# zju3dv/LoG

Hardware: NVIDIA H100
Metric: gaussians_per_s_fwd_bwd (higher is better)
Workload: dtype f32

## Files before the change

### log_b200/csrc/lgr_bin.cu

```cuda
#include "lgr_common.cuh"
#include "lgr_prof.cuh"

namespace lgr {

constexpr int SCAN_THREADS = 1024;
constexpr int SORT_CAP_SMALL_FWD = 4096;

__global__ void __launch_bounds__(SCAN_THREADS)
tile_scan_kernel(int ntiles, int32_t* __restrict__ tile_start ,
                 int32_t* __restrict__ cursor ,
                 int32_t* __restrict__ meta, int small_cap) {
  __shared__ int warp_sum[SCAN_THREADS / 32];
  __shared__ int carry_s, maxl_s, nbig_s;
  const int tid = threadIdx.x, lane = tid & 31, wid = tid >> 5;
  if (tid == 0) { carry_s = 0; maxl_s = 0; nbig_s = 0; }
  __syncthreads();
  int local_max = 0;
  for (int base = 0; base < ntiles; base += SCAN_THREADS) {
    const int i = base + tid;
    const int c = (i < ntiles) ? cursor[i * CSTRIDE] + cursor[i * CSTRIDE + 1] : 0;
    local_max = max(local_max, c);
    int x = c;
#pragma unroll
    for (int o = 1; o < 32; o <<= 1) { const int y = __shfl_up_sync(0xffffffffu, x, o); if (lane >= o) x += y; }
    if (lane == 31) warp_sum[wid] = x;
    __syncthreads();
    if (wid == 0) {
      int w = warp_sum[lane];
#pragma unroll
      for (int o = 1; o < 32; o <<= 1) { const int y = __shfl_up_sync(0xffffffffu, w, o); if (lane >= o) w += y; }
      warp_sum[lane] = w;
    }
    __syncthreads();
    const int carry = carry_s;
    const int excl = carry + (wid ? warp_sum[wid - 1] : 0) + x - c;
    if (i < ntiles) {
      tile_start[i] = excl; cursor[i * CSTRIDE] = 0;
      if (c > small_cap) cursor[CSTRIDE * ntiles + atomicAdd(&nbig_s, 1)] = i;
    }
    __syncthreads();
    if (tid == SCAN_THREADS - 1) carry_s = carry + warp_sum[31];
    __syncthreads();
  }
#pragma unroll
  for (int o = 16; o > 0; o >>= 1) local_max = max(local_max, __shfl_xor_sync(0xffffffffu, local_max, o));
  if (lane == 0) atomicMax(&maxl_s, local_max);
  __syncthreads();
  if (tid == 0) { tile_start[ntiles] = carry_s; meta[0] = carry_s; meta[1] = maxl_s; meta[5] = nbig_s; }
}

constexpr int BIN_THREADS = 256;
constexpr int PART_ROUNDS = 8;
constexpr int PLACE_GRID = 132 * 4;
constexpr int PART_CAP = 2048;
constexpr int PART_FLUSH_AT = PART_CAP - 4 * BIN_THREADS;
constexpr int PLACE_ITEMS = 8;
constexpr int PLACE_CHUNK = PLACE_ITEMS * BIN_THREADS;
#ifndef LGR_BIN_DIRECT_MAX
#define LGR_BIN_DIRECT_MAX (1 << 16)
#endif
constexpr int64_t BIN_DIRECT_MAX = LGR_BIN_DIRECT_MAX;
constexpr int PLACE_WINDOW = 2047;

__device__ __forceinline__ unsigned long long composite(uint32_t k, uint32_t v) { return ((unsigned long long)k << 32) | v; }

int part_smem_bytes(int rows) { return 3 * (int)sizeof(int32_t) * max(rows, 1); }

__device__ __forceinline__ void block_exclusive_scan(const int* in, int* out, int len, int* wsum) {
  const int tid = threadIdx.x, lane = tid & 31, wid = tid >> 5;
  int carry = 0;
  for (int base = 0; base < len; base += BIN_THREADS) {
    const int c = base + tid < len ? in[base + tid] : 0;
    int x = c;
#pragma unroll
    for (int o = 1; o < 32; o <<= 1) { const int y = __shfl_up_sync(0xffffffffu, x, o); if (lane >= o) x += y; }
    if (lane == 31) wsum[wid] = x;
    __syncthreads();
    int before = carry, all = carry;
#pragma unroll
    for (int w = 0; w < BIN_THREADS / 32; w++) { if (w < wid) before += wsum[w]; all += wsum[w]; }
    if (base + tid < len) out[base + tid] = before + x - c;
    carry = all;
    __syncthreads();
  }
}

__global__ void __launch_bounds__(BIN_THREADS, 6)
bin_partition_kernel(View v, int64_t n, const float* __restrict__ splat, const int32_t* __restrict__ radii,
                     const int32_t* __restrict__ tile_start, int32_t* __restrict__ cursor, unsigned long long* __restrict__ stage,
                     int32_t* __restrict__ stage_tile, int64_t capacity ,
                     int rounds ,
                     uint32_t* __restrict__ direct_key, uint32_t* __restrict__ direct_val ) {
  extern __shared__ int32_t row_tab[];
  __shared__ uint32_t s_key[PART_CAP], s_id[PART_CAP];
  __shared__ int32_t s_tile[PART_CAP];
  __shared__ uint16_t s_perm[PART_CAP];
  __shared__ int s_fill;
  __shared__ int s_wsum[BIN_THREADS / 32];
  __shared__ int64_t s_first[LGR_SHARD_MAX_RANKS + 1];
  const int rows = v.row1 - v.row0, lane = threadIdx.x & 31;
  int32_t* r_cnt = row_tab;
  int32_t* r_off = row_tab + rows;
  int32_t* r_base = row_tab + 2 * rows;
  for (int r = threadIdx.x; r < rows; r += BIN_THREADS) r_cnt[r] = 0;
  if (threadIdx.x == 0) s_fill = 0;
  const int64_t total = v.region_count ? region_setup(v, s_first) : n;
  __syncthreads();
  auto flush = [&]() {
    const int held = s_fill;
    if (direct_key) {
      for (int e = threadIdx.x; e < held; e += BIN_THREADS) {
        const int t = s_tile[e];
        const int64_t pos = (int64_t)tile_start[t] + atomicAdd(cursor + t * CSTRIDE, 1);
        if (pos < capacity) { direct_key[pos] = s_key[e]; direct_val[pos] = s_id[e]; }
      }
      __syncthreads();
      for (int r = threadIdx.x; r < rows; r += BIN_THREADS) r_cnt[r] = 0;
      if (threadIdx.x == 0) s_fill = 0;
      __syncthreads();
      return;
    }
    for (int r = threadIdx.x; r < rows; r += BIN_THREADS) {
      const int c = r_cnt[r];
      if (c > 0) r_base[r] = tile_start[r * v.gx] + atomicAdd(cursor + r * v.gx * CSTRIDE + 2, c);
    }
    block_exclusive_scan(r_cnt, r_off, rows, s_wsum);
    for (int r = threadIdx.x; r < rows; r += BIN_THREADS) r_base[r] -= r_off[r];
    __syncthreads();
    for (int e = threadIdx.x; e < held; e += BIN_THREADS) s_perm[atomicAdd(&r_off[s_tile[e] / v.gx], 1)] = (uint16_t)e;
    __syncthreads();
    for (int j = threadIdx.x; j < held; j += BIN_THREADS) {
      const int e = s_perm[j], t = s_tile[e];
      const int64_t pos = (int64_t)r_base[t / v.gx] + j;
      if (pos < capacity) { stage[pos] = composite(s_key[e], s_id[e]); stage_tile[pos] = t; }
    }
    __syncthreads();
    for (int r = threadIdx.x; r < rows; r += BIN_THREADS) r_cnt[r] = 0;
    if (threadIdx.x == 0) s_fill = 0;
    __syncthreads();
  };
  for (int64_t chunk = (int64_t)blockIdx.x * rounds * BIN_THREADS; chunk < total; chunk += (int64_t)gridDim.x * rounds * BIN_THREADS) {
    for (int round = 0; round < rounds; round++) {
      int64_t i = chunk + round * BIN_THREADS + threadIdx.x;
      bool live = i < total;
      if (live && v.region_count) i = region_row(v, s_first, i);
      if (live && v.num_owners > 0) {
        const int b = (int)(i / 256), sl = (int)(i % 256);
        if (sl >= v.band_blk[b]) live = false;
        else {
          const int id = v.band_ids[i];
          v.band_rows[v.band_blk[v.band_blocks + b] + sl] = id;
          if (v.band_dsplat) {
            float4* z = reinterpret_cast<float4*>(v.band_dsplat + (int64_t)id * LGR_GRAD_FLOATS);
            z[0] = z[1] = z[2] = make_float4(0.f, 0.f, 0.f, 0.f);
          }
          i = id;
        }
      }
      int rad = 0;
      float4 r0 = make_float4(0.f, 0.f, 0.f, 0.f), r1 = r0;
      float depth = 0.f;
      if (live) {
        rad = radii[i];
        r0 = ldg4(splat + i * LGR_SPLAT_FLOATS);
        r1 = ldg4(splat + i * LGR_SPLAT_FLOATS + 4);
        depth = __ldg(splat + i * LGR_SPLAT_FLOATS + 11);
        live = rad > 0;
      }
      if (live && v.num_owners == 0 && v.band_dsplat) {
        float4* z = reinterpret_cast<float4*>(v.band_dsplat + i * LGR_GRAD_FLOATS);
        z[0] = z[1] = z[2] = make_float4(0.f, 0.f, 0.f, 0.f);
      }
      int x0 = 0, y0 = 0, x1 = 0, y1 = 0;
      uint32_t key = 0;
      if (live) {
        live = r1.z > 0.f;
        if (live) {
          key = __float_as_uint(depth);
          tile_rect_tight(r0.x, r0.y, rad, r1.z, r1.w, v.gx, v.gy, v.row0, v.row1, x0, y0, x1, y1);
        }
      }
      const int w = x1 - x0, cnt = live ? w * (y1 - y0) : 0;
      const int mine = cnt <= 4 ? cnt : 0;
      int incl = mine;
#pragma unroll
      for (int o = 1; o < 32; o <<= 1) { const int y = __shfl_up_sync(0xffffffffu, incl, o); if (lane >= o) incl += y; }
      int wbase = 0;
      if (lane == 31 && incl > 0) wbase = atomicAdd(&s_fill, incl);
      wbase = __shfl_sync(0xffffffffu, wbase, 31);
      for (int k = 0, s = wbase + incl - mine; k < mine; k++, s++) {
        const int ty = y0 + k / w, tx = x0 + k % w;
        s_key[s] = key; s_id[s] = (uint32_t)i; s_tile[s] = (ty - v.row0) * v.gx + tx;
        atomicAdd(&r_cnt[ty - v.row0], 1);
      }
      unsigned todo = __ballot_sync(0xffffffffu, cnt > 4);
      while (todo) {
        const int src = __ffs(todo) - 1;
        todo &= todo - 1;
        const int bx0 = __shfl_sync(0xffffffffu, x0, src), by0 = __shfl_sync(0xffffffffu, y0, src);
        const int bw = __shfl_sync(0xffffffffu, w, src), bcnt = __shfl_sync(0xffffffffu, cnt, src);
        const uint32_t bkey = __shfl_sync(0xffffffffu, key, src);
        const uint32_t bid = (uint32_t)__shfl_sync(0xffffffffu, (int)i, src);
        const int bh = bcnt / bw;
        if (direct_key) {
          for (int k = lane; k < bcnt; k += 32) {
            const int t = (by0 + k / bw - v.row0) * v.gx + bx0 + k % bw;
            const int64_t pos = (int64_t)tile_start[t] + atomicAdd(cursor + t * CSTRIDE, 1);
            if (pos < capacity) { direct_key[pos] = bkey; direct_val[pos] = bid; }
          }
          continue;
        }
        for (int ry = 0; ry < bh; ry += 32) {
          const int nr = min(32, bh - ry), r_lane = by0 + ry + lane - v.row0;
          int rb = 0;
          if (lane < nr) rb = tile_start[r_lane * v.gx] + atomicAdd(cursor + r_lane * v.gx * CSTRIDE + 2, bw);
          for (int k0 = 0; k0 < nr * bw; k0 += 32) {
            const int k = k0 + lane;
            const int p = __shfl_sync(0xffffffffu, rb, k < nr * bw ? k / bw : 0);
            if (k < nr * bw) {
              const int64_t pos = (int64_t)p + k % bw;
              if (pos < capacity) {
                stage[pos] = composite(bkey, bid);
                stage_tile[pos] = (by0 + ry + k / bw - v.row0) * v.gx + bx0 + k % bw;
              }
            }
          }
        }
      }
      __syncthreads();
      if (__syncthreads_or(s_fill > (round == rounds - 1 ? 0 : PART_FLUSH_AT))) flush();
    }
  }
}

__global__ void __launch_bounds__(BIN_THREADS)
bin_place_kernel(int gx, int ntiles, const int32_t* __restrict__ tile_start, int32_t* __restrict__ cursor,
                 const unsigned long long* __restrict__ stage, const int32_t* __restrict__ stage_tile, uint32_t* __restrict__ inst_key,
                 uint32_t* __restrict__ inst_val) {
  constexpr int PER = (PLACE_WINDOW + 1) / BIN_THREADS;
  static_assert(PER * BIN_THREADS == PLACE_WINDOW + 1, "bucket count");
  __shared__ int s_cnt[PLACE_WINDOW + 1];
  __shared__ int s_base[PLACE_WINDOW];
  __shared__ unsigned long long s_e[PLACE_CHUNK];
  __shared__ uint16_t s_b[PLACE_CHUNK];
  __shared__ int s_wsum[BIN_THREADS / 32];
  __shared__ int s_t0;
  const int lane = threadIdx.x & 31, wid = threadIdx.x >> 5;
  const int total = tile_start[ntiles];
  for (int beg = blockIdx.x * PLACE_CHUNK; beg < total; beg += gridDim.x * PLACE_CHUNK) {
    for (int j = threadIdx.x; j <= PLACE_WINDOW; j += BIN_THREADS) s_cnt[j] = 0;
    if (threadIdx.x == 0) s_t0 = stage_tile[beg] - stage_tile[beg] % gx;
    __syncthreads();
    const int t0 = s_t0;
    int tk[PLACE_ITEMS], rank[PLACE_ITEMS];
#pragma unroll
    for (int k = 0; k < PLACE_ITEMS; k++) {
      const int idx = beg + k * BIN_THREADS + threadIdx.x;
      tk[k] = idx < total ? stage_tile[idx] : -1;
    }
#pragma unroll
    for (int k = 0; k < PLACE_ITEMS; k++) {
      rank[k] = 0;
      if (tk[k] >= 0) {
        const int b = min(tk[k] - t0, PLACE_WINDOW);
        rank[k] = b < PLACE_WINDOW ? atomicAdd(&s_cnt[b], 1) : tile_start[tk[k]] + atomicAdd(cursor + tk[k] * CSTRIDE, 1);
        tk[k] = b;
      }
    }
    __syncthreads();
    int c[PER], sum = 0;
    const int b0 = threadIdx.x * PER;
    int32_t* const cur = cursor + (int64_t)(t0 + b0) * CSTRIDE;
#pragma unroll
    for (int q = 0; q < PER; q++) {
      c[q] = s_cnt[b0 + q];
      sum += c[q];
    }
#pragma unroll
    for (int q = 0; q < PER; q++)
      if (c[q] > 0 && b0 + q < PLACE_WINDOW) s_base[b0 + q] = tile_start[t0 + b0 + q] + atomicAdd(cur + q * CSTRIDE, c[q]);
    int x = sum;
#pragma unroll
    for (int o = 1; o < 32; o <<= 1) { const int y = __shfl_up_sync(0xffffffffu, x, o); if (lane >= o) x += y; }
    if (lane == 31) s_wsum[wid] = x;
    __syncthreads();
    int off = x - sum;
#pragma unroll
    for (int w = 0; w < BIN_THREADS / 32; w++) if (w < wid) off += s_wsum[w];
#pragma unroll
    for (int q = 0; q < PER; q++) {
      const int b = threadIdx.x * PER + q;
      s_cnt[b] = off;
      if (b < PLACE_WINDOW && c[q] > 0) s_base[b] -= off;
      off += c[q];
    }
    __syncthreads();
#pragma unroll
    for (int k = 0; k < PLACE_ITEMS; k++) {
      if (tk[k] >= 0) {
        const unsigned long long e = stage[beg + k * BIN_THREADS + threadIdx.x];
        const int b = tk[k];
        if (b < PLACE_WINDOW) {
          const int j = s_cnt[b] + rank[k];
          s_e[j] = e; s_b[j] = (uint16_t)b;
        } else {
          inst_key[rank[k]] = (uint32_t)(e >> 32); inst_val[rank[k]] = (uint32_t)e;
        }
      }
    }
    __syncthreads();
    const int inside = s_cnt[PLACE_WINDOW];
    for (int j = threadIdx.x; j < inside; j += BIN_THREADS) {
      const int pos = s_base[s_b[j]] + j;
      const unsigned long long e = s_e[j];
      inst_key[pos] = (uint32_t)(e >> 32); inst_val[pos] = (uint32_t)e;
    }
    __syncthreads();
  }
}

constexpr int SORT_THREADS = 256;
constexpr int SORT_WARPS = SORT_THREADS / 32;
constexpr int RADIX_BITS = 8;
constexpr int RADIX = 1 << RADIX_BITS;
constexpr int SORT_CAP_SMALL = SORT_CAP_SMALL_FWD;
constexpr int SORT_CAP_LARGE = 13312;

__device__ __forceinline__ bool radix_pass(const uint32_t* __restrict__ kin, const uint32_t* __restrict__ vin,
                                           uint32_t* __restrict__ kout, uint32_t* __restrict__ vout, int len, int shift,
                                           bool on_val, int* __restrict__ whist) {
  const int tid = threadIdx.x, lane = tid & 31, wid = tid >> 5;
  const int seg = ((len + SORT_WARPS * 32 - 1) / (SORT_WARPS * 32)) * 32;
  const int beg = min(len, wid * seg), end = min(len, beg + seg);
  for (int j = tid; j < SORT_WARPS * RADIX; j += SORT_THREADS) whist[j] = 0;
  __syncthreads();
  int* myh = whist + wid * RADIX;
  for (int i = beg + lane; i < end; i += 32) {
    const uint32_t d = ((on_val ? vin[i] : kin[i]) >> shift) & (RADIX - 1);
    atomicAdd(myh + d, 1);
  }
  __syncthreads();
  {
    const int d = tid;
    int tot = 0;
#pragma unroll
    for (int w = 0; w < SORT_WARPS; w++) tot += whist[w * RADIX + d];
    int x = tot;
#pragma unroll
    for (int o = 1; o < 32; o <<= 1) { const int y = __shfl_up_sync(0xffffffffu, x, o); if (lane >= o) x += y; }
    __shared__ int wsum[SORT_WARPS];
    if (lane == 31) wsum[wid] = x;
    __syncthreads();
    int base = x - tot;
#pragma unroll
    for (int w = 0; w < SORT_WARPS; w++) if (w < wid) base += wsum[w];
#pragma unroll
    for (int w = 0; w < SORT_WARPS; w++) { const int c = whist[w * RADIX + d]; whist[w * RADIX + d] = base; base += c; }
    if (__syncthreads_or(tot == len)) return true;
  }
  for (int i0 = beg; i0 < end; i0 += 32) {
    const int i = i0 + lane;
    const bool ok = i < end;
    uint32_t k = 0, val = 0;
    if (ok) { k = kin[i]; val = vin[i]; }
    const uint32_t d = ok ? (((on_val ? val : k) >> shift) & (RADIX - 1)) : (RADIX + lane);
    const uint32_t peers = __match_any_sync(0xffffffffu, d);
    const int rank = __popc(peers & ((1u << lane) - 1u));
    int base = 0;
    if (ok) base = myh[d];
    __syncwarp();
    if (ok && rank == 0) myh[d] = base + __popc(peers);
    __syncwarp();
    if (ok) { kout[base + rank] = k; vout[base + rank] = val; }
  }
  __syncthreads();
  return false;
}

__device__ __forceinline__ void sort_tile(uint32_t* kA, uint32_t* vA, uint32_t* kB, uint32_t* vB, int len, int id_bits,
                                          int* whist) {
  uint32_t *ki = kA, *vi = vA, *ko = kB, *vo = vB;
  auto run = [&](int shift, bool on_val) {
    const bool ident = radix_pass(ki, vi, ko, vo, len, shift, on_val, whist);
    if (!ident) { uint32_t* t = ki; ki = ko; ko = t; t = vi; vi = vo; vo = t; }
  };
  for (int s = 0; s < 32; s += RADIX_BITS) run(s, false);
  int my_tie = 0;
  for (int i = threadIdx.x + 1; i < len; i += SORT_THREADS) if (ki[i] == ki[i - 1]) my_tie = 1;
  if (__syncthreads_or(my_tie)) {
    for (int s = 0; s < id_bits; s += RADIX_BITS) run(s, true);
    for (int s = 0; s < 32; s += RADIX_BITS) run(s, false);
  }
  if (ki != kA) {
    for (int i = threadIdx.x; i < len; i += SORT_THREADS) { kA[i] = ki[i]; vA[i] = vi[i]; }
    __syncthreads();
  }
}

#ifndef LGR_ON_LSD_FALLBACK
#define LGR_ON_LSD_FALLBACK()
#endif
constexpr int MSD_SMALL = 96;
constexpr int MSD_STACK = 512;

struct MsdShared {
  int hist[RADIX];
  int bstart[RADIX + 1];
  alignas(16) int wsum[SORT_WARPS];
  unsigned long long wmin[SORT_WARPS], wmax[SORT_WARPS];
  int stack_beg[MSD_STACK], stack_len[MSD_STACK];
  int top, shift, overflow;
};

__device__ __forceinline__ bool sort_tile_msd(uint32_t* kA, uint32_t* vA, uint32_t* kB, uint32_t* vB, int len, MsdShared& sh) {
  const int tid = threadIdx.x, lane = tid & 31, wid = tid >> 5;
  if (tid == 0) { sh.stack_beg[0] = 0; sh.stack_len[0] = len; sh.top = 1; sh.overflow = 0; }
  __syncthreads();
  while (true) {
    const int top = sh.top;
    if (top == 0 || sh.overflow) break;
    const int beg = sh.stack_beg[top - 1], n = sh.stack_len[top - 1];
    __syncthreads();
    if (tid == 0) sh.top = top - 1;
    unsigned long long mn = ~0ull, mx = 0ull;
    for (int i = tid; i < n; i += SORT_THREADS) {
      const unsigned long long c = composite(kA[beg + i], vA[beg + i]);
      mn = min(mn, c); mx = max(mx, c);
    }
#pragma unroll
    for (int o = 16; o > 0; o >>= 1) {
      mn = min(mn, __shfl_xor_sync(0xffffffffu, mn, o));
      mx = max(mx, __shfl_xor_sync(0xffffffffu, mx, o));
    }
    if (lane == 0) { sh.wmin[wid] = mn; sh.wmax[wid] = mx; }
    sh.hist[tid] = 0;
    __syncthreads();
    if (tid == 0) {
      unsigned long long a = sh.wmin[0], b = sh.wmax[0];
#pragma unroll
      for (int w = 1; w < SORT_WARPS; w++) { a = min(a, sh.wmin[w]); b = max(b, sh.wmax[w]); }
      const int hb = 63 - __clzll((long long)(a ^ b));
      sh.shift = max(0, hb - (RADIX_BITS - 1));
    }
    __syncthreads();
    const int shift = sh.shift;
    for (int i = tid; i < n; i += SORT_THREADS)
      atomicAdd(&sh.hist[(int)((composite(kA[beg + i], vA[beg + i]) >> shift) & (RADIX - 1))], 1);
    __syncthreads();
    {
      const int c = sh.hist[tid];
      int x = c;
#pragma unroll
      for (int o = 1; o < 32; o <<= 1) { const int y = __shfl_up_sync(0xffffffffu, x, o); if (lane >= o) x += y; }
      if (lane == 31) sh.wsum[wid] = x;
      __syncthreads();
      int base = x - c;
#pragma unroll
      for (int w = 0; w < SORT_WARPS; w++) if (w < wid) base += sh.wsum[w];
      sh.bstart[tid] = base;
      sh.hist[tid] = base;
      if (tid == RADIX - 1) sh.bstart[RADIX] = base + c;
    }
    __syncthreads();
    for (int i = tid; i < n; i += SORT_THREADS) {
      const uint32_t k = kA[beg + i], v = vA[beg + i];
      const int slot = atomicAdd(&sh.hist[(int)((composite(k, v) >> shift) & (RADIX - 1))], 1);
      kB[beg + slot] = k; vB[beg + slot] = v;
    }
    __syncthreads();
    for (int i = tid; i < n; i += SORT_THREADS) {
      const uint32_t k = kB[beg + i], v = vB[beg + i];
      const int d = (int)((composite(k, v) >> shift) & (RADIX - 1));
      const int b0 = sh.bstart[d], bn = sh.bstart[d + 1] - b0;
      int dst = i;
      if (bn <= MSD_SMALL) {
        const uint32_t* kb = kB + beg + b0;
        const uint32_t* vb = vB + beg + b0;
        int rank = 0, eq = 0;
#pragma unroll 8
        for (int j = 0; j < bn; j++) {
          const uint32_t kj = kb[j];
          rank += (kj < k) ? 1 : 0;
          eq += (kj == k) ? 1 : 0;
        }
        if (eq > 1)
          for (int j = 0; j < bn; j++) rank += (kb[j] == k && vb[j] < v) ? 1 : 0;
        dst = b0 + rank;
      }
      kA[beg + dst] = k; vA[beg + dst] = v;
    }
    {
      const int b0 = sh.bstart[tid], bn = sh.bstart[tid + 1] - b0;
      if (bn > MSD_SMALL) {
        const int slot = atomicAdd(&sh.top, 1);
        if (slot < MSD_STACK) { sh.stack_beg[slot] = beg + b0; sh.stack_len[slot] = bn; }
        else sh.overflow = 1;
      }
    }
    __syncthreads();
  }
  const bool ok = sh.overflow == 0;
  __syncthreads();
  return ok;
}

template <int MODE>
__global__ void __launch_bounds__(SORT_THREADS)
tile_sort_kernel(const int32_t* __restrict__ tile_list ,
                 const int32_t* __restrict__ tile_start, uint32_t* __restrict__ inst_key,
                 uint32_t* __restrict__ inst_val, uint32_t* __restrict__ tmp, int32_t* __restrict__ sorted_ids, int lo,
                 int cap, int id_bits, const int32_t* __restrict__ count_ptr) {
  extern __shared__ uint32_t smem_u32[];
  __shared__ int whist_s[MODE == 1 ? SORT_WARPS * RADIX : 1];
  int* const whist = MODE == 2 ? reinterpret_cast<int*>(smem_u32) : whist_s;
  __shared__ MsdShared msd;
  const int count = count_ptr ? *count_ptr : (int)gridDim.x;
  for (int b = blockIdx.x; b < count; b += gridDim.x) {
    const int t = tile_list ? tile_list[b] : b;
    const int beg = tile_start[t], len = tile_start[t + 1] - beg;
    if (len <= lo) continue;
    if (MODE == 0 && len > cap) continue;
    if (MODE != 1 && len <= cap) {
      uint32_t* kA = smem_u32; uint32_t* vA = kA + cap; uint32_t* kB = vA + cap; uint32_t* vB = kB + cap;
      for (int i = threadIdx.x; i < len; i += SORT_THREADS) { kA[i] = inst_key[beg + i]; vA[i] = inst_val[beg + i]; }
      __syncthreads();
      if (len > 1 && !sort_tile_msd(kA, vA, kB, vB, len, msd)) __trap();
      for (int i = threadIdx.x; i < len; i += SORT_THREADS) sorted_ids[beg + i] = (int32_t)vA[i];
    } else {
      uint32_t* kA = inst_key + beg; uint32_t* vA = inst_val + beg;
      uint32_t* kB = tmp + 2 * (int64_t)beg; uint32_t* vB = kB + len;
      __syncthreads();
      if (!sort_tile_msd(kA, vA, kB, vB, len, msd)) {
        LGR_ON_LSD_FALLBACK();
        sort_tile(kA, vA, kB, vB, len, id_bits, whist);
      }
      for (int i = threadIdx.x; i < len; i += SORT_THREADS) sorted_ids[beg + i] = (int32_t)vA[i];
    }
    __syncthreads();
  }
}

__global__ void __launch_bounds__(256)
clamp_lists_kernel(int ntiles, int64_t capacity, int32_t* __restrict__ tile_start, int32_t* __restrict__ meta) {
  const int flags = ((int64_t)meta[0] > capacity ? 1 : 0) | (meta[1] > LGR_CONTRIB_MAX_LIST ? 2 : 0);
  if (!flags) return;
  for (int i = blockIdx.x * 256 + threadIdx.x; i <= ntiles; i += gridDim.x * 256) tile_start[i] = 0;
  if (blockIdx.x == 0 && threadIdx.x == 0) atomicOr(meta + 6, flags);
}


int sort_smem_capacity() { return SORT_CAP_LARGE; }

constexpr int PC_THREADS = 1024;

__global__ void __launch_bounds__(PC_THREADS)
pc_block_count_kernel(int64_t n, const int32_t* __restrict__ count, int32_t* __restrict__ blk) {
  const int64_t i = (int64_t)blockIdx.x * PC_THREADS + threadIdx.x;
  const int c = __syncthreads_count(i < n && count[i] > 0);
  if (threadIdx.x == 0) blk[blockIdx.x] = c;
}

__global__ void __launch_bounds__(1024)
pc_scan_kernel(int nb, int32_t* __restrict__ blk , int32_t* __restrict__ num_out) {
  __shared__ int warp_sum[32];
  __shared__ int carry_s;
  const int tid = threadIdx.x, lane = tid & 31, wid = tid >> 5;
  if (tid == 0) carry_s = 0;
  __syncthreads();
  for (int base = 0; base < nb; base += 1024) {
    const int b = base + tid;
    const int c = b < nb ? blk[b] : 0;
    int x = c;
#pragma unroll
    for (int o = 1; o < 32; o <<= 1) { const int y = __shfl_up_sync(0xffffffffu, x, o); if (lane >= o) x += y; }
    if (lane == 31) warp_sum[wid] = x;
    __syncthreads();
    if (wid == 0) {
      int w = warp_sum[lane];
#pragma unroll
      for (int o = 1; o < 32; o <<= 1) { const int y = __shfl_up_sync(0xffffffffu, w, o); if (lane >= o) w += y; }
      warp_sum[lane] = w;
    }
    __syncthreads();
    const int carry = carry_s;
    if (b < nb) blk[nb + b] = carry + (wid ? warp_sum[wid - 1] : 0) + x - c;
    __syncthreads();
    if (tid == 1023) carry_s = carry + warp_sum[31];
    __syncthreads();
  }
  if (tid == 0) { blk[2 * nb] = carry_s; *num_out = carry_s; }
}

__global__ void __launch_bounds__(PC_THREADS)
pc_compact_kernel(int64_t n, const int32_t* __restrict__ count, const int32_t* __restrict__ blk, int nb,
                  int32_t* __restrict__ ids_out, int32_t* __restrict__ counts_out) {
  __shared__ int wsum[PC_THREADS / 32];
  const int64_t i = (int64_t)blockIdx.x * PC_THREADS + threadIdx.x;
  const int lane = threadIdx.x & 31, wid = threadIdx.x >> 5;
  const int c = i < n ? count[i] : 0;
  const unsigned bal = __ballot_sync(0xffffffffu, c > 0);
  if (lane == 0) wsum[wid] = __popc(bal);
  __syncthreads();
  int base = blk[nb + blockIdx.x];
  for (int w = 0; w < wid; w++) base += wsum[w];
  if (c > 0) {
    const int pos = base + __popc(bal & ((1u << lane) - 1u));
    ids_out[pos] = (int32_t)i;
    counts_out[pos] = c;
  }
}

int launch_point_compact(int64_t n, const int32_t* count, int32_t* blk, int32_t* ids_out, int32_t* counts_out, int32_t* num_out,
                         cudaStream_t st) {
  const int nb = (int)((n + PC_THREADS - 1) / PC_THREADS);
  if (nb == 0) {
    cudaError_t e = cudaMemsetAsync(num_out, 0, sizeof(int32_t), st);
    return e == cudaSuccess ? 0 : (int)e;
  }
  pc_block_count_kernel<<<nb, PC_THREADS, 0, st>>>(n, count, blk);
  LGR_CHECK_LAUNCH();
  pc_scan_kernel<<<1, 1024, 0, st>>>(nb, blk, num_out);
  LGR_CHECK_LAUNCH();
  pc_compact_kernel<<<nb, PC_THREADS, 0, st>>>(n, count, blk, nb, ids_out, counts_out);
  LGR_CHECK_LAUNCH();
  return 0;
}

int launch_tile_scan(int ntiles, int32_t* tile_start, int32_t* cursor, int32_t* meta, bool , cudaStream_t st) {
  ProfScope ps(K_TILE_SCAN, st);
  tile_scan_kernel<<<1, SCAN_THREADS, 0, st>>>(ntiles, tile_start, cursor, meta, SORT_CAP_SMALL_FWD);
  LGR_CHECK_LAUNCH();
  return 0;
}

constexpr int LONG_SORT_GRID = 132;

int launch_bin_and_sort(const View& v, int64_t n, int64_t num_inst, int max_len, int num_long, const float* splat,
                        const int32_t* radii, int32_t* tile_start, int32_t* cursor, uint32_t* inst_key,
                        uint32_t* inst_val, uint32_t* inst_tmp, int32_t* sorted_ids, int32_t* meta_dev, cudaStream_t st) {
  if (n == 0) return 0;
  if (meta_dev) {
    const int nt = v.gx * (v.row1 - v.row0);
    clamp_lists_kernel<<<(nt + 256) / 256, 256, 0, st>>>(nt, num_inst, tile_start, meta_dev);
    LGR_CHECK_LAUNCH();
  }
  if (num_inst == 0 && v.num_owners == 0 && v.band_dsplat == nullptr) return 0;
  if (num_inst > 0 && (!inst_tmp || !sorted_ids)) return LGR_E_BADARG;
  const int ntiles = v.gx * (v.row1 - v.row0);
  const int part_smem = part_smem_bytes(v.row1 - v.row0);
  if (part_smem > 160 * 1024) return LGR_E_UNSUPPORTED;
  {
    cudaError_t e = cudaFuncSetAttribute(bin_partition_kernel, cudaFuncAttributeMaxDynamicSharedMemorySize, part_smem);
    if (e != cudaSuccess) return (int)e;
  }
  const int rounds = (int)max((int64_t)1, min((int64_t)PART_ROUNDS, n / ((int64_t)BIN_THREADS * 132 * 16)));
  const int64_t chunk = (int64_t)rounds * BIN_THREADS;
  unsigned blocks = (unsigned)((n + chunk - 1) / chunk);
  if (v.region_count && blocks > (unsigned)LGR_REGION_GRID) blocks = (unsigned)LGR_REGION_GRID;
  unsigned long long* stage = reinterpret_cast<unsigned long long*>(inst_tmp);
  {
    ProfScope ps(K_BIN_SCATTER, st, num_inst > BIN_DIRECT_MAX ? 2 : 1);
    const bool direct = num_inst <= BIN_DIRECT_MAX;
    bin_partition_kernel<<<blocks, BIN_THREADS, part_smem, st>>>(v, n, splat, radii, tile_start, cursor, stage, sorted_ids, num_inst,
                                                                 rounds, direct ? inst_key : nullptr, direct ? inst_val : nullptr);
    LGR_CHECK_LAUNCH();
    if (num_inst > 0 && !direct) {
      const unsigned place = (unsigned)min((int64_t)PLACE_GRID, (num_inst + PLACE_CHUNK - 1) / PLACE_CHUNK);
      bin_place_kernel<<<place, BIN_THREADS, 0, st>>>(v.gx, ntiles, tile_start, cursor, stage, sorted_ids, inst_key, inst_val);
      LGR_CHECK_LAUNCH();
    }
  }
  if (num_inst == 0) return 0;
  int id_bits = 8;
  while (id_bits < 32 && (n - 1) >> id_bits) id_bits += 8;
  {
    cudaError_t e = cudaFuncSetAttribute(tile_sort_kernel<0>, cudaFuncAttributeMaxDynamicSharedMemorySize, 16 * SORT_CAP_LARGE);
    if (e == cudaSuccess && meta_dev) e = cudaFuncSetAttribute(tile_sort_kernel<2>, cudaFuncAttributeMaxDynamicSharedMemorySize, 16 * SORT_CAP_LARGE);
    if (e != cudaSuccess) return (int)e;
  }
  if (meta_dev) {
    ProfScope ps(K_TILE_SORT, st, 2);
    tile_sort_kernel<0><<<ntiles, SORT_THREADS, 16 * SORT_CAP_SMALL, st>>>(nullptr, tile_start, inst_key, inst_val, inst_tmp, sorted_ids, 0, SORT_CAP_SMALL, id_bits, nullptr);
    LGR_CHECK_LAUNCH();
    const int32_t* long_list = cursor + CSTRIDE * ntiles;
    tile_sort_kernel<2><<<LONG_SORT_GRID, SORT_THREADS, 16 * SORT_CAP_LARGE, st>>>(long_list, tile_start, inst_key, inst_val, inst_tmp, sorted_ids, SORT_CAP_SMALL, SORT_CAP_LARGE, id_bits, meta_dev + 5);
    LGR_CHECK_LAUNCH();
    return 0;
  }
  ProfScope ps(K_TILE_SORT, st, 1 + (num_long > 0) + (max_len > SORT_CAP_LARGE));
  const int cap_main = max(256, min(max_len, SORT_CAP_SMALL));
  tile_sort_kernel<0><<<ntiles, SORT_THREADS, 16 * cap_main, st>>>(nullptr, tile_start, inst_key, inst_val, inst_tmp, sorted_ids, 0, cap_main, id_bits, nullptr);
  LGR_CHECK_LAUNCH();
  if (num_long > 0) {
    const int32_t* long_list = cursor + CSTRIDE * ntiles;
    const int cap = min(max_len, SORT_CAP_LARGE);
    tile_sort_kernel<0><<<num_long, SORT_THREADS, 16 * cap, st>>>(long_list, tile_start, inst_key, inst_val, inst_tmp, sorted_ids, SORT_CAP_SMALL, cap, id_bits, nullptr);
    LGR_CHECK_LAUNCH();
    if (max_len > SORT_CAP_LARGE) {
      tile_sort_kernel<1><<<num_long, SORT_THREADS, 0, st>>>(long_list, tile_start, inst_key, inst_val, inst_tmp, sorted_ids, SORT_CAP_LARGE, 0, id_bits, nullptr);
      LGR_CHECK_LAUNCH();
    }
  }
  return 0;
}

}
```

Baseline: 1.931 billion.

## Sort tile lists in registers with bucket sort and wider long-list blocks

Replaces the shared-memory MSD radix sort for tiles that fit on chip with a register-resident bucket sort. It uses 4×threads range-mapped buckets plus in-bin rank counting, and writes sorted ids straight to global memory. Long lists now use 512-thread blocks, and dynamic shared memory per entry drops from 16 to 10 bytes, which should raise occupancy and cut global/shared traffic. The change also adds compile-time probe modes and a split-benchmark script, and risks register pressure from the per-thread item arrays and deeper recursion for skewed key distributions.

```diff
diff --git a/log_b200/csrc/lgr_bin.cu b/log_b200/csrc/lgr_bin.cu
--- a/log_b200/csrc/lgr_bin.cu
+++ b/log_b200/csrc/lgr_bin.cu
@@ -320,19 +320,23 @@
 }
 
 constexpr int SORT_THREADS = 256;
-constexpr int SORT_WARPS = SORT_THREADS / 32;
+constexpr int LONG_SORT_THREADS = 512;
 constexpr int RADIX_BITS = 8;
 constexpr int RADIX = 1 << RADIX_BITS;
 constexpr int SORT_CAP_SMALL = SORT_CAP_SMALL_FWD;
 constexpr int SORT_CAP_LARGE = 13312;
-
+constexpr int SORT_SMEM_PER_ENTRY = 10;
+
+template <int THREADS>
 __device__ __forceinline__ bool radix_pass(const uint32_t* __restrict__ kin, const uint32_t* __restrict__ vin,
                                            uint32_t* __restrict__ kout, uint32_t* __restrict__ vout, int len, int shift,
                                            bool on_val, int* __restrict__ whist) {
+  constexpr int WARPS = THREADS / 32;
+  static_assert(THREADS >= RADIX, "one thread per digit in the scan");
   const int tid = threadIdx.x, lane = tid & 31, wid = tid >> 5;
-  const int seg = ((len + SORT_WARPS * 32 - 1) / (SORT_WARPS * 32)) * 32;
+  const int seg = ((len + WARPS * 32 - 1) / (WARPS * 32)) * 32;
   const int beg = min(len, wid * seg), end = min(len, beg + seg);
-  for (int j = tid; j < SORT_WARPS * RADIX; j += SORT_THREADS) whist[j] = 0;
+  for (int j = tid; j < WARPS * RADIX; j += THREADS) whist[j] = 0;
   __syncthreads();
   int* myh = whist + wid * RADIX;
   for (int i = beg + lane; i < end; i += 32) {
@@ -343,20 +347,23 @@
   {
     const int d = tid;
     int tot = 0;
-#pragma unroll
-    for (int w = 0; w < SORT_WARPS; w++) tot += whist[w * RADIX + d];
+    if (d < RADIX)
+#pragma unroll
+      for (int w = 0; w < WARPS; w++) tot += whist[w * RADIX + d];
     int x = tot;
 #pragma unroll
     for (int o = 1; o < 32; o <<= 1) { const int y = __shfl_up_sync(0xffffffffu, x, o); if (lane >= o) x += y; }
-    __shared__ int wsum[SORT_WARPS];
-    if (lane == 31) wsum[wid] = x;
-    __syncthreads();
-    int base = x - tot;
-#pragma unroll
-    for (int w = 0; w < SORT_WARPS; w++) if (w < wid) base += wsum[w];
-#pragma unroll
-    for (int w = 0; w < SORT_WARPS; w++) { const int c = whist[w * RADIX + d]; whist[w * RADIX + d] = base; base += c; }
-    if (__syncthreads_or(tot == len)) return true;
+    __shared__ int wsum[RADIX / 32];
+    if (lane == 31 && d < RADIX) wsum[wid] = x;
+    __syncthreads();
+    if (d < RADIX) {
+      int base = x - tot;
+#pragma unroll
+      for (int w = 0; w < RADIX / 32; w++) if (w < wid) base += wsum[w];
+#pragma unroll
+      for (int w = 0; w < WARPS; w++) { const int c = whist[w * RADIX + d]; whist[w * RADIX + d] = base; base += c; }
+    }
+    if (__syncthreads_or(d < RADIX && tot == len)) return true;
   }
   for (int i0 = beg; i0 < end; i0 += 32) {
     const int i = i0 + lane;
@@ -377,24 +384,34 @@
   return false;
 }
 
+template <int THREADS>
 __device__ __forceinline__ void sort_tile(uint32_t* kA, uint32_t* vA, uint32_t* kB, uint32_t* vB, int len, int id_bits,
                                           int* whist) {
   uint32_t *ki = kA, *vi = vA, *ko = kB, *vo = vB;
   auto run = [&](int shift, bool on_val) {
-    const bool ident = radix_pass(ki, vi, ko, vo, len, shift, on_val, whist);
+    const bool ident = radix_pass<THREADS>(ki, vi, ko, vo, len, shift, on_val, whist);
     if (!ident) { uint32_t* t = ki; ki = ko; ko = t; t = vi; vi = vo; vo = t; }
   };
   for (int s = 0; s < 32; s += RADIX_BITS) run(s, false);
   int my_tie = 0;
-  for (int i = threadIdx.x + 1; i < len; i += SORT_THREADS) if (ki[i] == ki[i - 1]) my_tie = 1;
+  for (int i = threadIdx.x + 1; i < len; i += THREADS) if (ki[i] == ki[i - 1]) my_tie = 1;
   if (__syncthreads_or(my_tie)) {
     for (int s = 0; s < id_bits; s += RADIX_BITS) run(s, true);
     for (int s = 0; s < 32; s += RADIX_BITS) run(s, false);
   }
   if (ki != kA) {
-    for (int i = threadIdx.x; i < len; i += SORT_THREADS) { kA[i] = ki[i]; vA[i] = vi[i]; }
-    __syncthreads();
-  }
+    for (int i = threadIdx.x; i < len; i += THREADS) { kA[i] = ki[i]; vA[i] = vi[i]; }
+    __syncthreads();
+  }
+}
+
+#ifndef LGR_SORT_PROBE
+#define LGR_SORT_PROBE 0
+#endif
+__device__ __forceinline__ uint32_t probe_key(uint32_t i) {
+  uint32_t h = i * 0x9e3779b9u;
+  h ^= h >> 16; h *= 0x85ebca6bu; h ^= h >> 13;
+  return __float_as_uint(2.f + 18.f * (float)(h >> 8) * (1.f / 16777216.f));
 }
 
 #ifndef LGR_ON_LSD_FALLBACK
@@ -403,16 +420,154 @@
 constexpr int MSD_SMALL = 96;
 constexpr int MSD_STACK = 512;
 
+__device__ __forceinline__ int rank_in_bin(const uint32_t* kb, const uint32_t* vb, int bn, uint32_t k, uint32_t v) {
+  int rank = 0, eq = 0;
+#pragma unroll 8
+  for (int j = 0; j < bn; j++) {
+    const uint32_t kj = kb[j];
+    rank += (kj < k) ? 1 : 0;
+    eq += (kj == k) ? 1 : 0;
+  }
+  if (eq > 1)
+    for (int j = 0; j < bn; j++) rank += (kb[j] == k && vb[j] < v) ? 1 : 0;
+  return rank;
+}
+
+struct BucketMap {
+  unsigned long long lo, mul;
+  int shift;
+  __device__ __forceinline__ int operator()(unsigned long long c) const { return (int)((((c - lo) >> shift) * mul) >> 32); }
+};
+
+__device__ __forceinline__ BucketMap bucket_map(unsigned long long lo, unsigned long long hi, int nb) {
+  const unsigned long long r = hi - lo;
+  const int shift = max(0, 32 - __clzll((long long)r));
+  return {lo, ((unsigned long long)nb << 32) / ((r >> shift) + 1), shift};
+}
+
+template <int THREADS>
+struct BucketShared {
+  static constexpr int NB = 4 * THREADS;
+  static_assert(NB % THREADS == 0, "whole buckets per thread in the scan");
+  static constexpr int STACK = (THREADS == SORT_THREADS ? SORT_CAP_SMALL : SORT_CAP_LARGE) / (MSD_SMALL + 1) + 1;
+  int start[NB + 1];
+  int wsum[THREADS / 32];
+  unsigned long long wmin[THREADS / 32], wmax[THREADS / 32];
+  int stack_beg[STACK], stack_len[STACK];
+  int top;
+};
+
+template <int THREADS, int ITEMS>
+__device__ __forceinline__ void sort_tile_shared(const uint32_t* __restrict__ gk, const uint32_t* __restrict__ gv, int len,
+                                                 uint32_t* K, uint32_t* V, uint16_t* OFF, int32_t* __restrict__ out,
+                                                 BucketShared<THREADS>& sh, int gbeg) {
+  constexpr int WARPS = THREADS / 32, NB = BucketShared<THREADS>::NB;
+  const int tid = threadIdx.x, lane = tid & 31, wid = tid >> 5;
+  uint32_t k[ITEMS], v[ITEMS];
+#pragma unroll
+  for (int j = 0; j < ITEMS; j++) {
+    if (j * THREADS >= len) break;
+    const int i = j * THREADS + tid;
+    if (i < len) {
+      if (LGR_SORT_PROBE == 2) { k[j] = probe_key(gbeg + i); v[j] = (uint32_t)i; }
+      else { k[j] = gk[i]; v[j] = gv[i]; }
+    }
+  }
+  if (LGR_SORT_PROBE == 1) {
+#pragma unroll
+    for (int j = 0; j < ITEMS && j * THREADS < len; j++) if (j * THREADS + tid < len) out[j * THREADS + tid] = (int32_t)v[j];
+    return;
+  }
+  if (tid == 0) sh.top = 0;
+  int b = 0, n = len;
+  while (true) {
+    unsigned long long mn = ~0ull, mx = 0ull;
+#pragma unroll
+    for (int j = 0; j < ITEMS && j * THREADS < n; j++)
+      if (j * THREADS + tid < n) { const unsigned long long c = composite(k[j], v[j]); mn = min(mn, c); mx = max(mx, c); }
+#pragma unroll
+    for (int o = 16; o > 0; o >>= 1) {
+      mn = min(mn, __shfl_xor_sync(0xffffffffu, mn, o));
+      mx = max(mx, __shfl_xor_sync(0xffffffffu, mx, o));
+    }
+    if (lane == 0) { sh.wmin[wid] = mn; sh.wmax[wid] = mx; }
+    for (int d = tid; d < NB; d += THREADS) sh.start[d] = 0;
+    __syncthreads();
+#pragma unroll
+    for (int w = 0; w < WARPS; w++) { mn = min(mn, sh.wmin[w]); mx = max(mx, sh.wmax[w]); }
+    const BucketMap map = bucket_map(mn, mx, NB);
+#pragma unroll
+    for (int j = 0; j < ITEMS && j * THREADS < n; j++) {
+      const int i = j * THREADS + tid;
+      if (i < n) OFF[i] = (uint16_t)atomicAdd(&sh.start[map(composite(k[j], v[j]))], 1);
+    }
+    __syncthreads();
+    {
+      constexpr int PER = NB / THREADS;
+      int c[PER], own = 0;
+#pragma unroll
+      for (int q = 0; q < PER; q++) { c[q] = sh.start[tid * PER + q]; own += c[q]; }
+      int x = own;
+#pragma unroll
+      for (int o = 1; o < 32; o <<= 1) { const int y = __shfl_up_sync(0xffffffffu, x, o); if (lane >= o) x += y; }
+      if (lane == 31) sh.wsum[wid] = x;
+      __syncthreads();
+      int base = x - own;
+#pragma unroll
+      for (int w = 0; w < WARPS; w++) if (w < wid) base += sh.wsum[w];
+#pragma unroll
+      for (int q = 0; q < PER; q++) { sh.start[tid * PER + q] = base; base += c[q]; }
+      if (tid == THREADS - 1) sh.start[NB] = base;
+    }
+    __syncthreads();
+#pragma unroll
+    for (int j = 0; j < ITEMS && j * THREADS < n; j++) {
+      const int i = j * THREADS + tid;
+      if (i < n) {
+        const int slot = b + sh.start[map(composite(k[j], v[j]))] + OFF[i];
+        K[slot] = k[j]; V[slot] = v[j];
+      }
+    }
+    __syncthreads();
+    for (int i = tid; i < n; i += THREADS) {
+      const uint32_t kk = K[b + i], vv = V[b + i];
+      const int d = map(composite(kk, vv));
+      const int b0 = sh.start[d], bn = sh.start[d + 1] - b0;
+      if (bn <= MSD_SMALL) out[b + b0 + rank_in_bin(K + b + b0, V + b + b0, bn, kk, vv)] = (int32_t)vv;
+    }
+    for (int d = tid; d < NB; d += THREADS) {
+      const int b0 = sh.start[d], bn = sh.start[d + 1] - b0;
+      if (bn > MSD_SMALL) {
+        const int s = atomicAdd(&sh.top, 1);
+        sh.stack_beg[s] = b + b0; sh.stack_len[s] = bn;
+      }
+    }
+    __syncthreads();
+    const int top = sh.top;
+    if (top == 0) break;
+    b = sh.stack_beg[top - 1]; n = sh.stack_len[top - 1];
+#pragma unroll
+    for (int j = 0; j < ITEMS && j * THREADS < n; j++)
+      if (j * THREADS + tid < n) { k[j] = K[b + j * THREADS + tid]; v[j] = V[b + j * THREADS + tid]; }
+    __syncthreads();
+    if (tid == 0) sh.top = top - 1;
+  }
+}
+
+template <int THREADS>
 struct MsdShared {
   int hist[RADIX];
   int bstart[RADIX + 1];
-  alignas(16) int wsum[SORT_WARPS];
-  unsigned long long wmin[SORT_WARPS], wmax[SORT_WARPS];
+  alignas(16) int wsum[RADIX / 32];
+  unsigned long long wmin[THREADS / 32], wmax[THREADS / 32];
   int stack_beg[MSD_STACK], stack_len[MSD_STACK];
   int top, shift, overflow;
 };
 
-__device__ __forceinline__ bool sort_tile_msd(uint32_t* kA, uint32_t* vA, uint32_t* kB, uint32_t* vB, int len, MsdShared& sh) {
+template <int THREADS>
+__device__ __forceinline__ bool sort_tile_msd(uint32_t* kA, uint32_t* vA, uint32_t* kB, uint32_t* vB, int len, MsdShared<THREADS>& sh) {
+  constexpr int WARPS = THREADS / 32;
+  static_assert(THREADS >= RADIX, "one thread per digit");
   const int tid = threadIdx.x, lane = tid & 31, wid = tid >> 5;
   if (tid == 0) { sh.stack_beg[0] = 0; sh.stack_len[0] = len; sh.top = 1; sh.overflow = 0; }
   __syncthreads();
@@ -423,7 +578,7 @@
     __syncthreads();
     if (tid == 0) sh.top = top - 1;
     unsigned long long mn = ~0ull, mx = 0ull;
-    for (int i = tid; i < n; i += SORT_THREADS) {
+    for (int i = tid; i < n; i += THREADS) {
       const unsigned long long c = composite(kA[beg + i], vA[beg + i]);
       mn = min(mn, c); mx = max(mx, c);
     }
@@ -433,63 +588,51 @@
       mx = max(mx, __shfl_xor_sync(0xffffffffu, mx, o));
     }
     if (lane == 0) { sh.wmin[wid] = mn; sh.wmax[wid] = mx; }
-    sh.hist[tid] = 0;
+    if (tid < RADIX) sh.hist[tid] = 0;
     __syncthreads();
     if (tid == 0) {
       unsigned long long a = sh.wmin[0], b = sh.wmax[0];
 #pragma unroll
-      for (int w = 1; w < SORT_WARPS; w++) { a = min(a, sh.wmin[w]); b = max(b, sh.wmax[w]); }
+      for (int w = 1; w < WARPS; w++) { a = min(a, sh.wmin[w]); b = max(b, sh.wmax[w]); }
       const int hb = 63 - __clzll((long long)(a ^ b));
       sh.shift = max(0, hb - (RADIX_BITS - 1));
     }
     __syncthreads();
     const int shift = sh.shift;
-    for (int i = tid; i < n; i += SORT_THREADS)
+    for (int i = tid; i < n; i += THREADS)
       atomicAdd(&sh.hist[(int)((composite(kA[beg + i], vA[beg + i]) >> shift) & (RADIX - 1))], 1);
     __syncthreads();
     {
-      const int c = sh.hist[tid];
+      const int c = tid < RADIX ? sh.hist[tid] : 0;
       int x = c;
 #pragma unroll
       for (int o = 1; o < 32; o <<= 1) { const int y = __shfl_up_sync(0xffffffffu, x, o); if (lane >= o) x += y; }
-      if (lane == 31) sh.wsum[wid] = x;
+      if (lane == 31 && tid < RADIX) sh.wsum[wid] = x;
       __syncthreads();
-      int base = x - c;
-#pragma unroll
-      for (int w = 0; w < SORT_WARPS; w++) if (w < wid) base += sh.wsum[w];
-      sh.bstart[tid] = base;
-      sh.hist[tid] = base;
-      if (tid == RADIX - 1) sh.bstart[RADIX] = base + c;
-    }
-    __syncthreads();
-    for (int i = tid; i < n; i += SORT_THREADS) {
+      if (tid < RADIX) {
+        int base = x - c;
+#pragma unroll
+        for (int w = 0; w < RADIX / 32; w++) if (w < wid) base += sh.wsum[w];
+        sh.bstart[tid] = base;
+        sh.hist[tid] = base;
+        if (tid == RADIX - 1) sh.bstart[RADIX] = base + c;
+      }
+    }
+    __syncthreads();
+    for (int i = tid; i < n; i += THREADS) {
       const uint32_t k = kA[beg + i], v = vA[beg + i];
       const int slot = atomicAdd(&sh.hist[(int)((composite(k, v) >> shift) & (RADIX - 1))], 1);
       kB[beg + slot] = k; vB[beg + slot] = v;
     }
     __syncthreads();
-    for (int i = tid; i < n; i += SORT_THREADS) {
+    for (int i = tid; i < n; i += THREADS) {
       const uint32_t k = kB[beg + i], v = vB[beg + i];
       const int d = (int)((composite(k, v) >> shift) & (RADIX - 1));
       const int b0 = sh.bstart[d], bn = sh.bstart[d + 1] - b0;
-      int dst = i;
-      if (bn <= MSD_SMALL) {
-        const uint32_t* kb = kB + beg + b0;
-        const uint32_t* vb = vB + beg + b0;
-        int rank = 0, eq = 0;
-#pragma unroll 8
-        for (int j = 0; j < bn; j++) {
-          const uint32_t kj = kb[j];
-          rank += (kj < k) ? 1 : 0;
-          eq += (kj == k) ? 1 : 0;
-        }
-        if (eq > 1)
-          for (int j = 0; j < bn; j++) rank += (kb[j] == k && vb[j] < v) ? 1 : 0;
-        dst = b0 + rank;
-      }
+      const int dst = bn <= MSD_SMALL ? b0 + rank_in_bin(kB + beg + b0, vB + beg + b0, bn, k, v) : i;
       kA[beg + dst] = k; vA[beg + dst] = v;
     }
-    {
+    if (tid < RADIX) {
       const int b0 = sh.bstart[tid], bn = sh.bstart[tid + 1] - b0;
       if (bn > MSD_SMALL) {
         const int slot = atomicAdd(&sh.top, 1);
@@ -504,16 +647,17 @@
   return ok;
 }
 
-template <int MODE>
-__global__ void __launch_bounds__(SORT_THREADS)
+template <int MODE, int THREADS>
+__global__ void __launch_bounds__(THREADS, THREADS == SORT_THREADS ? 4 : 1)
 tile_sort_kernel(const int32_t* __restrict__ tile_list ,
                  const int32_t* __restrict__ tile_start, uint32_t* __restrict__ inst_key,
                  uint32_t* __restrict__ inst_val, uint32_t* __restrict__ tmp, int32_t* __restrict__ sorted_ids, int lo,
                  int cap, int id_bits, const int32_t* __restrict__ count_ptr) {
+  constexpr int ITEMS = (THREADS == SORT_THREADS ? SORT_CAP_SMALL : SORT_CAP_LARGE) / THREADS;
+  static_assert(ITEMS * THREADS == (THREADS == SORT_THREADS ? SORT_CAP_SMALL : SORT_CAP_LARGE), "cap in registers");
   extern __shared__ uint32_t smem_u32[];
-  __shared__ int whist_s[MODE == 1 ? SORT_WARPS * RADIX : 1];
+  __shared__ int whist_s[MODE == 1 ? (THREADS / 32) * RADIX : 1];
   int* const whist = MODE == 2 ? reinterpret_cast<int*>(smem_u32) : whist_s;
-  __shared__ MsdShared msd;
   const int count = count_ptr ? *count_ptr : (int)gridDim.x;
   for (int b = blockIdx.x; b < count; b += gridDim.x) {
     const int t = tile_list ? tile_list[b] : b;
@@ -521,20 +665,22 @@
     if (len <= lo) continue;
     if (MODE == 0 && len > cap) continue;
     if (MODE != 1 && len <= cap) {
-      uint32_t* kA = smem_u32; uint32_t* vA = kA + cap; uint32_t* kB = vA + cap; uint32_t* vB = kB + cap;
-      for (int i = threadIdx.x; i < len; i += SORT_THREADS) { kA[i] = inst_key[beg + i]; vA[i] = inst_val[beg + i]; }
-      __syncthreads();
-      if (len > 1 && !sort_tile_msd(kA, vA, kB, vB, len, msd)) __trap();
-      for (int i = threadIdx.x; i < len; i += SORT_THREADS) sorted_ids[beg + i] = (int32_t)vA[i];
-    } else {
+      if constexpr (MODE != 1) {
+        __shared__ BucketShared<THREADS> bsh;
+        uint32_t* K = smem_u32; uint32_t* V = K + cap;
+        uint16_t* OFF = reinterpret_cast<uint16_t*>(V + cap);
+        sort_tile_shared<THREADS, ITEMS>(inst_key + beg, inst_val + beg, len, K, V, OFF, sorted_ids + beg, bsh, beg);
+      }
+    } else if constexpr (MODE != 0) {
+      __shared__ MsdShared<THREADS> msd;
       uint32_t* kA = inst_key + beg; uint32_t* vA = inst_val + beg;
       uint32_t* kB = tmp + 2 * (int64_t)beg; uint32_t* vB = kB + len;
       __syncthreads();
-      if (!sort_tile_msd(kA, vA, kB, vB, len, msd)) {
+      if (!sort_tile_msd<THREADS>(kA, vA, kB, vB, len, msd)) {
         LGR_ON_LSD_FALLBACK();
-        sort_tile(kA, vA, kB, vB, len, id_bits, whist);
-      }
-      for (int i = threadIdx.x; i < len; i += SORT_THREADS) sorted_ids[beg + i] = (int32_t)vA[i];
+        sort_tile<THREADS>(kA, vA, kB, vB, len, id_bits, whist);
+      }
+      for (int i = threadIdx.x; i < len; i += THREADS) sorted_ids[beg + i] = (int32_t)vA[i];
     }
     __syncthreads();
   }
@@ -674,30 +820,31 @@
   int id_bits = 8;
   while (id_bits < 32 && (n - 1) >> id_bits) id_bits += 8;
   {
-    cudaError_t e = cudaFuncSetAttribute(tile_sort_kernel<0>, cudaFuncAttributeMaxDynamicSharedMemorySize, 16 * SORT_CAP_LARGE);
-    if (e == cudaSuccess && meta_dev) e = cudaFuncSetAttribute(tile_sort_kernel<2>, cudaFuncAttributeMaxDynamicSharedMemorySize, 16 * SORT_CAP_LARGE);
+    cudaError_t e = cudaFuncSetAttribute(tile_sort_kernel<0, SORT_THREADS>, cudaFuncAttributeMaxDynamicSharedMemorySize, SORT_SMEM_PER_ENTRY * SORT_CAP_SMALL);
+    if (e == cudaSuccess) e = cudaFuncSetAttribute(tile_sort_kernel<0, LONG_SORT_THREADS>, cudaFuncAttributeMaxDynamicSharedMemorySize, SORT_SMEM_PER_ENTRY * SORT_CAP_LARGE);
+    if (e == cudaSuccess && meta_dev) e = cudaFuncSetAttribute(tile_sort_kernel<2, LONG_SORT_THREADS>, cudaFuncAttributeMaxDynamicSharedMemorySize, SORT_SMEM_PER_ENTRY * SORT_CAP_LARGE);
     if (e != cudaSuccess) return (int)e;
   }
   if (meta_dev) {
     ProfScope ps(K_TILE_SORT, st, 2);
-    tile_sort_kernel<0><<<ntiles, SORT_THREADS, 16 * SORT_CAP_SMALL, st>>>(nullptr, tile_start, inst_key, inst_val, inst_tmp, sorted_ids, 0, SORT_CAP_SMALL, id_bits, nullptr);
+    tile_sort_kernel<0, SORT_THREADS><<<ntiles, SORT_THREADS, SORT_SMEM_PER_ENTRY * SORT_CAP_SMALL, st>>>(nullptr, tile_start, inst_key, inst_val, inst_tmp, sorted_ids, 0, SORT_CAP_SMALL, id_bits, nullptr);
     LGR_CHECK_LAUNCH();
     const int32_t* long_list = cursor + CSTRIDE * ntiles;
-    tile_sort_kernel<2><<<LONG_SORT_GRID, SORT_THREADS, 16 * SORT_CAP_LARGE, st>>>(long_list, tile_start, inst_key, inst_val, inst_tmp, sorted_ids, SORT_CAP_SMALL, SORT_CAP_LARGE, id_bits, meta_dev + 5);
+    tile_sort_kernel<2, LONG_SORT_THREADS><<<LONG_SORT_GRID, LONG_SORT_THREADS, SORT_SMEM_PER_ENTRY * SORT_CAP_LARGE, st>>>(long_list, tile_start, inst_key, inst_val, inst_tmp, sorted_ids, SORT_CAP_SMALL, SORT_CAP_LARGE, id_bits, meta_dev + 5);
     LGR_CHECK_LAUNCH();
     return 0;
   }
   ProfScope ps(K_TILE_SORT, st, 1 + (num_long > 0) + (max_len > SORT_CAP_LARGE));
   const int cap_main = max(256, min(max_len, SORT_CAP_SMALL));
-  tile_sort_kernel<0><<<ntiles, SORT_THREADS, 16 * cap_main, st>>>(nullptr, tile_start, inst_key, inst_val, inst_tmp, sorted_ids, 0, cap_main, id_bits, nullptr);
+  tile_sort_kernel<0, SORT_THREADS><<<ntiles, SORT_THREADS, SORT_SMEM_PER_ENTRY * cap_main, st>>>(nullptr, tile_start, inst_key, inst_val, inst_tmp, sorted_ids, 0, cap_main, id_bits, nullptr);
   LGR_CHECK_LAUNCH();
   if (num_long > 0) {
     const int32_t* long_list = cursor + CSTRIDE * ntiles;
     const int cap = min(max_len, SORT_CAP_LARGE);
-    tile_sort_kernel<0><<<num_long, SORT_THREADS, 16 * cap, st>>>(long_list, tile_start, inst_key, inst_val, inst_tmp, sorted_ids, SORT_CAP_SMALL, cap, id_bits, nullptr);
+    tile_sort_kernel<0, LONG_SORT_THREADS><<<num_long, LONG_SORT_THREADS, SORT_SMEM_PER_ENTRY * cap, st>>>(long_list, tile_start, inst_key, inst_val, inst_tmp, sorted_ids, SORT_CAP_SMALL, cap, id_bits, nullptr);
     LGR_CHECK_LAUNCH();
     if (max_len > SORT_CAP_LARGE) {
-      tile_sort_kernel<1><<<num_long, SORT_THREADS, 0, st>>>(long_list, tile_start, inst_key, inst_val, inst_tmp, sorted_ids, SORT_CAP_LARGE, 0, id_bits, nullptr);
+      tile_sort_kernel<1, SORT_THREADS><<<num_long, SORT_THREADS, 0, st>>>(long_list, tile_start, inst_key, inst_val, inst_tmp, sorted_ids, SORT_CAP_LARGE, 0, id_bits, nullptr);
       LGR_CHECK_LAUNCH();
     }
   }
diff --git a/profiles/sort_split_bench.py b/profiles/sort_split_bench.py
--- /dev/null
+++ b/profiles/sort_split_bench.py
@@ -0,0 +1,82 @@
+import argparse
+import json
+import os
+import shutil
+import statistics
+import subprocess
+import sys
+import tempfile
+
+ROOT = os.path.dirname(os.path.dirname(os.path.abspath(__file__)))
+VARIANTS = {'full': 0, 'no_sort': 1, 'synth_load': 2}
+
+
+def prepare(work, name, flag):
+    tree = os.path.join(work, name)
+    lib = os.path.join(tree, 'log_b200', '_lib', 'liblog_b200_raster.so')
+    if os.path.exists(lib):
+        return tree
+    os.makedirs(tree, exist_ok=True)
+    shutil.copy(os.path.join(ROOT, 'bench.py'), tree)
+    for d in ('log_b200', 'include'):
+        shutil.copytree(os.path.join(ROOT, d), os.path.join(tree, d), dirs_exist_ok=True,
+                        ignore=shutil.ignore_patterns('_lib', '__pycache__'))
+    env = dict(os.environ, LGR_NVCC_EXTRA=f'-DLGR_SORT_PROBE={flag}')
+    subprocess.check_call([sys.executable, '-c', 'from log_b200 import build; build.build(force=True)'], cwd=tree, env=env)
+    return tree
+
+
+def run(tree, workload, steps, warmup):
+    out = subprocess.run([sys.executable, os.path.join(tree, 'bench.py'), '--workload', workload, '--steps', str(steps),
+                          '--warmup', str(warmup), '--no-cpu-baseline', '--no-e2e'], cwd=tree, capture_output=True, text=True)
+    if out.returncode != 0:
+        raise SystemExit(out.stdout[-2000:] + out.stderr[-4000:])
+    line = json.loads([l for l in out.stdout.splitlines() if l.startswith('{')][-1])
+    return {'ms_per_step': line['ms_per_step'], 'tile_sort_ms': line['kernel_ms_bin_sort']['tile_sort'],
+            'instances': line['config']['instances_binned'], 'longest': line['config']['longest_tile_list']}
+
+
+def gpu_info():
+    q = 'name,power.limit,clocks.max.sm,clocks.sm'
+    r = subprocess.run(['nvidia-smi', f'--query-gpu={q}', '--format=csv,noheader'], capture_output=True, text=True)
+    return dict(zip(q.split(','), [s.strip() for s in r.stdout.splitlines()[0].split(',')])) if r.returncode == 0 else {}
+
+
+def main():
+    ap = argparse.ArgumentParser()
+    ap.add_argument('--workloads', nargs='+', default=['10m', 'big300k'])
+    ap.add_argument('--reps', type=int, default=3)
+    ap.add_argument('--steps', type=int, default=20)
+    ap.add_argument('--warmup', type=int, default=3)
+    ap.add_argument('--work', default=None, help='where the builds go (kept and reused if given; default: a temporary directory)')
+    ap.add_argument('--build-only', action='store_true')
+    ap.add_argument('--out', default=None)
+    args = ap.parse_args()
+    work = os.path.abspath(args.work) if args.work else tempfile.mkdtemp(prefix='lgr_sort_split_')
+    trees = {v: prepare(work, v, f) for v, f in VARIANTS.items()}
+    if args.build_only:
+        return
+    res = {'gpu': gpu_info(), 'steps': args.steps, 'warmup': args.warmup, 'workloads': {}}
+    for w in args.workloads:
+        runs = {v: [] for v in VARIANTS}
+        for _ in range(args.reps):
+            for v in VARIANTS:
+                runs[v].append(run(trees[v], w, args.steps, args.warmup))
+        summary = {}
+        for v, rs in runs.items():
+            t = [r['tile_sort_ms'] for r in rs]
+            summary[v] = {'tile_sort_ms_median': statistics.median(t), 'tile_sort_ms_range': [min(t), max(t)], 'runs': rs}
+        res['workloads'][w] = summary
+        print(w, {v: round(s['tile_sort_ms_median'], 4) for v, s in summary.items()}, flush=True)
+    res['gpu_after'] = gpu_info()
+    text = json.dumps(res, indent=1)
+    print(text)
+    if args.out:
+        with open(args.out, 'w') as f:
+            f.write(text + '\n')
+    if not args.work:
+        shutil.rmtree(work, ignore_errors=True)
+
+
+if __name__ == '__main__':
+    main()
```

Result: faster. 1.966 billion, median of 6 (+1.8%).
